# AI4REALNET/network-distributed-q-learning

Hardware: AMD Instinct MI355X
Metric: agent-env-steps/sec (whole node), 64-switch map, 1/2/4/8 MI355X vs CPU (higher is better)
Workload: dtype f64

## Files before the change

### network-distributed-q-learning_amd/csrc/sfl_core.h

```cpp
#pragma once
#include <stdint.h>
#include "sfl_rng.h"

#if !defined(__HIPCC__)
#include <math.h>
#endif

namespace sfl {

enum : uint32_t { A_NOTHING = 0, A_LEFT = 1, A_FWD = 2, A_RIGHT = 3, A_STOP = 4, A_NONE = 15 };
enum : uint32_t { S_WAITING = 0, S_READY = 1, S_MF_OFF = 2, S_MOVING = 3, S_STOPPED = 4, S_MALF = 5, S_DONE = 6 };
enum : int32_t { PH_RESET = 0, PH_TICK = 1, PH_DECIDE = 2, PH_POST = 3, PH_END = 4 };
enum : uint32_t { F_TERM = 1, F_TRUNC = 2, F_GREEDY = 4, F_EXPLOIT_DONE = 8, F_OWN_SCAN = 16, F_INFLIGHT = 32 };
enum : uint32_t { F_EXT_OBS = 128 };
enum : uint32_t {
  E_INF_DIST = 1,
  E_PLAN_OVF = 2,
  E_PORT = 4,
  E_BAD_ACTION = 8,
  E_LR_TABLE = 32,
};

constexpr int32_t DIST_INF = 0x3FFFFFFF;
constexpr int OWN_MAX = 16;
constexpr int MAXW = 4;
constexpr uint32_t PEND_NONE = 0xFFFFFFFFu;
constexpr uint16_t PORT_NONE = 0xFFFFu;

struct SflMap {
  int32_t H, W, S, T, K, NP, HW, cell_bits;
  int32_t max_episode_steps, mf_min, mf_max, ntab;
  int32_t delay_thr;
  double mf_rate, gamma, eps0, eps_decay, lr0, lr_decay, default_q;
  uint64_t mf_thresh, mf_magic;
  uint32_t mf_n;
  int64_t max_steps;
  uint64_t q_per_env;
  uint32_t rows_per_env, touched_words;
  const uint16_t* grid;
  const int16_t* cell_sw;
  const uint8_t* sw_np;
  const uint8_t* sw_na;
  const uint8_t* act_src;
  const uint8_t* act_dst;
  const uint8_t* act_turn;
  const uint8_t* act_j;
  const uint8_t* first_other;
  const uint8_t* port_side;
  const uint8_t* slot_nroutes;
  const uint8_t* slot_route_act;
  const uint8_t* q_w;
  const int16_t* port_nb;
  const int16_t* port_len;
  const int16_t* port_unique;
  const uint64_t* q_off;
  const uint32_t* row_base;
  const int32_t* dist;
  const int32_t* tr_ed;
  const int32_t* tr_la;
  const int32_t* tr_k;
  const int32_t* tr_target;
  const int32_t* tr_init_cell;
  const int32_t* tr_init_dist;
  const int32_t* tr_init_delay;
  const uint8_t* tr_init_dir;
  const int16_t* tr_init_port;
  const double* eps_tab;
  const double* lr_tab;
  const uint32_t* sw_pack;
  const uint32_t* port_pack;
  const uint32_t* move_tab;
  const uint32_t* move2c_tab;
  const int32_t* tr_pack;
  const uint32_t* seedseq32;
  const uint32_t* port_tr;
  const uint8_t* mf_tab;
  int32_t mf_steps;
  int32_t n_groups;
  const uint16_t* env_group;
  const double* hpg_eps_tab;
  const double* hpg_lr_tab;
  const double* hpg_sc;
};
enum : int { HPG_EPS0 = 0, HPG_EPS_DECAY = 1, HPG_LR0 = 2, HPG_LR_DECAY = 3 };

SFL_FN uint32_t mod_small(uint64_t x, uint32_t n, uint64_t M) {
#if defined(__HIP_DEVICE_COMPILE__)
  const uint64_t q = __umul64hi(x, M);
#else
  const uint64_t q = (uint64_t)(((unsigned __int128)x * M) >> 64);
#endif
  uint64_t r = x - q * (uint64_t)n;
  if (r >= n) r -= n;
  return (uint32_t)r;
}

inline void mf_prepare(SflMap& m) {
  const double R = ldexp(m.mf_rate, 53);
  m.mf_thresh = !(m.mf_rate > 0.0) ? 0ull : (R >= 9007199254740992.0 ? (1ull << 53) : (uint64_t)ceil(R));
  const int64_t n = (int64_t)m.mf_max - (int64_t)m.mf_min + 1;
  m.mf_n = (n >= 1 && n < (1ll << 32)) ? (uint32_t)n : 0u;
  m.mf_magic = m.mf_n ? ~0ull / m.mf_n : 0ull;
}

SFL_FN uint32_t mf_propose(const SflMap& m, uint64_t seed, uint32_t e, int32_t t, int h) {
  if (m.mf_steps > 0) {
    if (t < 1 || t > m.mf_steps) return 0u;
    return m.mf_tab[((size_t)e * (uint32_t)m.mf_steps + (uint32_t)(t - 1)) * (uint32_t)m.T + (uint32_t)h];
  }
  if (!(m.mf_rate > 0.0)) return 0u;
  const uint64_t z = mf_draw(seed, (uint64_t)t, (uint64_t)h);
  if ((z >> 11) >= m.mf_thresh) return 0u;
  const uint64_t x = mix64(z ^ 0xA0761D6478BD642Full);
  const uint32_t r = m.mf_n ? mod_small(x, m.mf_n, m.mf_magic)
                            : (uint32_t)(x % (uint64_t)(m.mf_max - m.mf_min + 1));
  return (uint32_t)(m.mf_min + (int32_t)r) + 1u;
}

struct SflState {
  uint32_t E;
  int32_t* phase;
  int32_t* elapsed;
  uint32_t* eflags;
  int32_t* ep_t;
  int32_t* n_test;
  uint32_t* epoch;
  uint64_t* rng;
  uint64_t* seed;
  double* cum_reward;
  int32_t* n_mf;
  int32_t* ep_dec;
  int32_t* ep_ticks;
  int64_t* step_ctr;
  int64_t* dec_total;
  uint32_t* masks;
  uint32_t* err;
  int32_t* tr_pos;
  uint32_t* tr_bits;
  uint32_t* tr_plan;
  uint16_t* tr_next;
  uint16_t* tr_prev;
  uint16_t* tr_src;
  uint16_t* tr_dec;
  int32_t* tr_delay;
  uint16_t* own;
  uint8_t* own_n;
  int32_t* sc_desired;
  int32_t* sc_pred;
  uint32_t* sc_aux;
  uint8_t* occ;
  uint8_t* claim;
  uint64_t* sem;
  uint64_t* slot;
  uint32_t* counts;
  double* q;
  uint32_t* touched;
};

struct SflCtl {
  int32_t mode;
  int32_t exploit_freq;
  int32_t ep_target;
  int32_t stats_cap;
  int32_t stats_base;
  int64_t dec_budget;
  double* st_cum;
  int32_t* st_arrived;
  int32_t* st_mf;
  int32_t* st_dec;
  int32_t* st_ticks;
  int32_t* st_delays;
  double* sx_cum;
  int32_t* sx_arrived;
  uint64_t* launch_dec;
  uint64_t* launch_ticks;
  uint64_t* launch_bytes;
  uint64_t* trace;
  uint64_t* trace_n;
  int32_t trace_env;
  int32_t trace_cap;
  const struct SflExt* ext;
  uint64_t* phase_cyc;
};

struct SflExt {
  const int32_t* actions;
  int32_t* agent;
  int32_t* train;
  int32_t* slot;
  uint32_t* state;
  uint32_t* mask;
  int32_t* reward;
  int32_t* now;
  int32_t* next_sw;
  int32_t* step_now;
  uint32_t* arrived;
  int32_t* n_mf;
  int32_t* delays;
  int32_t* truncated;
// ... 1248 lines not shown
```

### network-distributed-q-learning_amd/csrc/sfl_engine.h

```cpp
#pragma once
#include <stdint.h>
#include <stdio.h>
#include <stdlib.h>
#include <string.h>

#include <algorithm>
#include <string>
#include <vector>

#include "../../include/sfl.h"
#include "sfl_consensus.h"
#include "sfl_core.h"
#include "sfl_curve.h"
#include "sfl_mfgen.h"
#include "sfl_part.h"

namespace sfl {

static thread_local std::string g_last_error;

inline int fail(const std::string& msg) {
  g_last_error = msg;
  return -1;
}
// ... 626 lines not shown
  if (write) h->eblk_state = 0;
  return 0;
}

template <class B>
int scan_errors(Handle<B>* h) {
  if (!h->last_err) return 0;
  if (int rc = part_host_access(h, false)) return rc;
  std::vector<uint32_t> err(h->E);
  h->be.d2h(err.data(), h->st.err, h->E * 4);
  if (h->be.sync()) return fail(h->be.error());
  for (uint32_t e = 0; e < h->E; ++e)
    if (err[e]) {
      char buf[256];
      snprintf(buf, sizeof buf, "env %u: error flags 0x%x (1=inf distance, 2=plan overflow, 4=port mismatch, 8=bad action, "
               "16=message segment overflow, 32=decayed lr beyond the ntab table: raise ntab)",
               e, err[e]);
      return fail(buf);
    }
  return 0;
}

template <class B>
int check_errors(Handle<B>* h) {
  if (int rc = reduce_launch(h)) return rc;
  return scan_errors(h);
}

template <class B>
int run(Handle<B>* h, const SflCtl& c_in, sfl_run_args* args) {
  if (h->part.world) return fail("sfl_run: the handle is graph-partitioned; drive it with sfl_part_*");
  if (h->env_mode) return fail("sfl_run: the handle is in external-action mode (sfl_env_begin); drive it with sfl_env_step");
  const bool grouped = h->map.env_group != nullptr;
  if (grouped && args && args->trace && args->trace_cap > 0)
    return fail("sfl_run: a per-decision trace is not available on a handle with hyperparameter groups");
  SflCtl c = c_in;
  const size_t E = h->E, T = h->map.T;
  const int32_t cap = args ? args->stats_cap : 0;
  std::vector<void*> scratch;
  auto scr = [&](size_t bytes) -> void* {
    void* p = h->be.alloc(bytes ? bytes : 1);
    scratch.push_back(p);
    return p;
  };
  c.stats_cap = cap;
  c.stats_base = c_in.stats_base;
  if (args && cap > 0) {
    c.st_cum = (double*)scr((size_t)cap * E * 8);
    c.st_arrived = (int32_t*)scr((size_t)cap * E * 4);
    c.st_mf = (int32_t*)scr((size_t)cap * E * 4);
    c.st_dec = (int32_t*)scr((size_t)cap * E * 4);
    c.st_ticks = (int32_t*)scr((size_t)cap * E * 4);
    c.st_delays = (int32_t*)scr((size_t)cap * T * E * 4);
    c.sx_cum = (double*)scr((size_t)cap * E * 8);
    c.sx_arrived = (int32_t*)scr((size_t)cap * E * 4);
    for (void* p : scratch)
      if (!p) {
        for (void* q : scratch) h->be.free(q);
        return fail("sfl_run: stats allocation failed");
      }
    h->be.memset(c.sx_cum, 0, (size_t)cap * E * 8);
    h->be.memset(c.sx_arrived, 0, (size_t)cap * E * 4);
  }
  const bool curve = !args && h->cv.on;
  if (curve) {
    const CurveArgs& a = h->cv.a;
    c.stats_cap = a.ring_cap;
    c.stats_base = 0;
    c.st_cum = const_cast<double*>(a.st_cum);
    c.st_arrived = const_cast<int32_t*>(a.st_arrived);
    c.st_mf = const_cast<int32_t*>(a.st_mf);
    c.st_dec = const_cast<int32_t*>(a.st_dec);
    c.st_ticks = const_cast<int32_t*>(a.st_ticks);
    c.st_delays = const_cast<int32_t*>(a.st_delays);
  }
  const bool xfold = curve && h->cv.x_on;
  if (xfold) {
    c.sx_cum = const_cast<double*>(h->cv.xa.sx_cum);
    c.sx_arrived = const_cast<int32_t*>(h->cv.xa.sx_arrived);
  }
  c.launch_dec = h->d_launch_dec;
  c.launch_ticks = h->d_launch_ticks;
  c.launch_bytes = h->d_launch_bytes;
  c.phase_cyc = args && !grouped ? h->d_phase : nullptr;
  uint64_t* d_trace = nullptr;
  uint64_t* d_trace_n = nullptr;
  if (args && args->trace && args->trace_cap > 0) {
    d_trace = (uint64_t*)scr((size_t)args->trace_cap * 32);
    d_trace_n = (uint64_t*)scr(8);
    if (!d_trace || !d_trace_n) {
      for (void* q : scratch) h->be.free(q);
      return fail("sfl_run: trace allocation failed");
    }
    h->be.memset(d_trace_n, 0, 8);
    c.trace = d_trace;
    c.trace_n = d_trace_n;
    c.trace_env = args->trace_env;
    c.trace_cap = args->trace_cap;
  }
  float ms = 0.f;
  int rc = h->be.run(h->map, h->st, c, h->variant, &ms);
  h->last_kernel_ms = ms;
  if (!rc && curve) rc = h->be.curve(h->cv.a, false);
  if (!rc && xfold) rc = h->be.curve_exploit(h->cv.xa, false);
  if (!rc && args && cap > 0) {
    if (args->cum_reward) h->be.d2h(args->cum_reward, c.st_cum, (size_t)cap * E * 8);
    if (args->arrived) h->be.d2h(args->arrived, c.st_arrived, (size_t)cap * E * 4);
    if (args->malfunctions) h->be.d2h(args->malfunctions, c.st_mf, (size_t)cap * E * 4);
    if (args->decisions) h->be.d2h(args->decisions, c.st_dec, (size_t)cap * E * 4);
    if (args->ticks) h->be.d2h(args->ticks, c.st_ticks, (size_t)cap * E * 4);
    if (args->delays) h->be.d2h(args->delays, c.st_delays, (size_t)cap * T * E * 4);
    if (args->exploit_cum) h->be.d2h(args->exploit_cum, c.sx_cum, (size_t)cap * E * 8);
    if (args->exploit_arrived) h->be.d2h(args->exploit_arrived, c.sx_arrived, (size_t)cap * E * 4);
  }
  if (!rc && d_trace) {
    h->be.d2h(args->trace_n, d_trace_n, 8);
    h->be.d2h(args->trace, d_trace, (size_t)args->trace_cap * 32);
  }
  if (!rc) rc = h->be.sync();
  for (void* p : scratch) h->be.free(p);
  if (rc) return fail(std::string("sfl_run: ") + h->be.error());
  if (curve) {
    h->cv.last_ms = h->be.elapsed_ms();
    h->cv.x_last_ms = xfold ? h->be.elapsed_exploit_ms() : 0.f;
    h->cv.last_ms += h->cv.x_last_ms;
    h->cv.total_ms += h->cv.last_ms;
    h->cv.x_total_ms += h->cv.x_last_ms;
  }
  return check_errors(h);
}

inline int ext_variant(int v) {
  if (v <= 0 || !kVariants[v].LM) return v;
  for (int u = 1; u < kNumVariants; ++u) {
    const WaveShape &a = kVariants[u], &b = kVariants[v];
    if (!a.LM && a.PPL == b.PPL && a.SPL == b.SPL && a.TW == b.TW && a.G == b.G) return u;
  }
  return 0;
}

template <class B>
int env_begin(Handle<B>* h, bool wave = false) {
  const std::string fn = wave ? "sfl_env_begin_wave" : "sfl_env_begin";
  if (h->part.world) return fail(fn + ": the handle is graph-partitioned");
  if (h->map.env_group) return fail(fn + ": the handle has hyperparameter groups (sfl_set_hparam_groups)");
  int variant = 0;
  if (wave) {
    if (!B::kHasWave)
      return fail(fn + ": this build has no wave kernels (the host build runs the lane-per-env body only)");
    variant = ext_variant(h->created_variant);
    if (variant <= 0)
      return fail(fn + ": the handle has no wave shape (" +
                  (h->variant_note.empty() ? std::string("SFL_KERNEL=scalar") : h->variant_note) + ")");
  }
  const size_t E = h->E, T = h->map.T, S = h->map.S, NP = h->map.NP;
  if (!h->d_ext) {
    SflExt& x = h->ext;
    x.actions = h->template dalloc<int32_t>(E);
    x.agent = h->template dalloc<int32_t>(E);
    x.train = h->template dalloc<int32_t>(E);
    x.slot = h->template dalloc<int32_t>(E);
    x.state = h->template dalloc<uint32_t>(E);
    x.mask = h->template dalloc<uint32_t>(E);
    x.reward = h->template dalloc<int32_t>(E);
    x.now = h->template dalloc<int32_t>(E);
    x.next_sw = h->template dalloc<int32_t>(E);
    x.step_now = h->template dalloc<int32_t>(E);
// ... 792 lines not shown
```

### network-distributed-q-learning_amd/csrc/sfl_rng.h

```cpp
#pragma once
#include <stdint.h>

#ifndef SFL_FN
#if defined(__HIPCC__)
#define SFL_FN __host__ __device__ inline __attribute__((always_inline))
#else
#define SFL_FN inline
#endif
#endif

namespace sfl {

struct Pcg64 {
  uint64_t shi, slo;
  uint64_t ihi, ilo;
  uint32_t has;
  uint32_t buf;
};

SFL_FN uint64_t mulhi64(uint64_t a, uint64_t b) {
#if defined(__HIP_DEVICE_COMPILE__)
  return __umul64hi(a, b);
#else
  return (uint64_t)(((unsigned __int128)a * b) >> 64);
// ... 23 lines not shown
    return g.buf;
  }
  uint64_t v = pcg_next64(g);
  g.has = 1;
  g.buf = (uint32_t)(v >> 32);
  return (uint32_t)v;
}

SFL_FN double pcg_double(Pcg64& g) { return (double)(pcg_next64(g) >> 11) * (1.0 / 9007199254740992.0); }

SFL_FN uint32_t pcg_bounded(Pcg64& g, uint32_t rng) {
  if (rng == 0) return 0;
  if (rng == 0xFFFFFFFFu) return pcg_next32(g);
  const uint32_t excl = rng + 1u;
  uint64_t m = (uint64_t)pcg_next32(g) * excl;
  uint32_t left = (uint32_t)m;
  if (left < excl) {
    const uint32_t thr = (0xFFFFFFFFu - rng) % excl;
    while (left < thr) {
      m = (uint64_t)pcg_next32(g) * excl;
      left = (uint32_t)m;
    }
  }
  return (uint32_t)(m >> 32);
}

SFL_FN void pcg_from_seedseq(uint32_t value, Pcg64& g) {
  uint32_t hc = 0x43b0d7e5u;
  uint32_t pool[4];
  for (int i = 0; i < 4; ++i) {
    uint32_t v = (i == 0) ? value : 0u;
    v ^= hc;
    hc *= 0x931e8875u;
    v *= hc;
    v ^= v >> 16;
    pool[i] = v;
  }
  for (int src = 0; src < 4; ++src) {
    for (int dst = 0; dst < 4; ++dst) {
      if (src == dst) continue;
      uint32_t v = pool[src];
      v ^= hc;
      hc *= 0x931e8875u;
      v *= hc;
      v ^= v >> 16;
      uint32_t r = 0xca01f9ddu * pool[dst] - 0x4973f715u * v;
      r ^= r >> 16;
      pool[dst] = r;
    }
  }
  uint32_t w[8];
  uint32_t hb = 0x8b51f9ddu;
  for (int i = 0; i < 8; ++i) {
    uint32_t d = pool[i & 3];
    d ^= hb;
    hb *= 0x58f38dedu;
    d *= hb;
    d ^= d >> 16;
    w[i] = d;
  }
  const uint64_t s_hi = (uint64_t)w[0] | ((uint64_t)w[1] << 32);
  const uint64_t s_lo = (uint64_t)w[2] | ((uint64_t)w[3] << 32);
  const uint64_t q_hi = (uint64_t)w[4] | ((uint64_t)w[5] << 32);
  const uint64_t q_lo = (uint64_t)w[6] | ((uint64_t)w[7] << 32);
  g.ihi = (q_hi << 1) | (q_lo >> 63);
  g.ilo = (q_lo << 1) | 1ull;
  g.shi = 0;
  g.slo = 0;
  pcg_step(g);
  uint64_t lo = g.slo + s_lo;
  g.shi = g.shi + s_hi + (lo < g.slo ? 1ull : 0ull);
  g.slo = lo;
  pcg_step(g);
  g.has = 0;
  g.buf = 0;
}

SFL_FN uint64_t mix64(uint64_t z) {
  z = (z ^ (z >> 30)) * 0xBF58476D1CE4E5B9ull;
  z = (z ^ (z >> 27)) * 0x94D049BB133111EBull;
  return z ^ (z >> 31);
}

SFL_FN uint64_t mf_draw(uint64_t seed, uint64_t tick, uint64_t handle) {
  return mix64(seed * 0x9E3779B97F4A7C15ull + tick * 0xD1B54A32D192ED03ull + handle * 0x8CB92BA72F3D8DD7ull +
               0x632BE59BD9B4E019ull);
}

}
```

### network-distributed-q-learning_amd/csrc/sfl_wave.h

```cpp
#pragma once
#include <hip/hip_runtime.h>

#include <type_traits>

#include "sfl_core.h"
#include "sfl_part.h"
#include "sfl_experiment.h"

namespace sfl {
namespace wave {

#ifndef SFL_PF_RING
#define SFL_PF_RING 12
#endif
#ifndef SFL_PF_RING64
#define SFL_PF_RING64 16
#endif
#ifndef SFL_TICK_HOLD
#define SFL_TICK_HOLD 2
#endif
#ifndef SFL_TICK_REMMIN
#define SFL_TICK_REMMIN 5
#endif

// ... 854 lines not shown
          w[0] = mk;
          w[1] = 0ull;
        } else {
          w[0] = mk.w[0];
          w[1] = mk.w[1];
        }
#pragma unroll
        for (int j = 0; j < 2 * NWD; ++j) st(s.masks, (size_t)(k * MAXW + j) * E + e, (uint32_t)(w[j >> 1] >> (32 * (j & 1))));
      };
      put(0, q_mask);
      put(1, arr_mask);
      put(2, fl_mask);
      put(3, mf_mask);
      if constexpr (!EXT) {
        st(s.rng, ix(0), lrng[0]);
        st(s.rng, ix(1), lrng[1]);
        st(s.rng, ix(4), lrng[4]);
      }
      st(s.cum_reward, e, (double)cum);
      st(s.n_mf, e, n_mf);
      st(s.ep_dec, e, ep_dec);
      st(s.ep_ticks, e, ep_ticks);
      st(s.step_ctr, e, (int64_t)step_ctr);
      st(s.dec_total, e, ld(s.dec_total, e) + (int64_t)n_dec);
    }
    return err;
  }
  __device__ __forceinline__ void store_eblk(int32_t phase, uint32_t err, int32_t ep_t, int32_t n_test, int64_t dec_done,
                                             int32_t req_dst, uint32_t upd_n, uint64_t l_dec, uint64_t l_ticks,
                                             uint64_t l_bytes) {
    if constexpr (PART) {
      uint32_t* sg = lsem0;
      auto put4 = [&](int i, uint32_t a, uint32_t b, uint32_t c, uint32_t d) {
        u4 v;
        v[0] = a;
        v[1] = b;
        v[2] = c;
        v[3] = d;
        *(u4*)(sg + i) = v;
      };
      auto lo = [](uint64_t x) { return (uint32_t)x; };
      auto hi = [](uint64_t x) { return (uint32_t)(x >> 32); };
      const uint64_t dtot = ebw64(EB_DEC_TOTAL) + (uint64_t)n_dec;
      const uint64_t cumd = (uint64_t)__double_as_longlong((double)cum);
      const uint64_t r0 = lrng[0], r1 = lrng[1], r2 = lrng[2], r3 = lrng[3], r4 = lrng[4];
      uint64_t mw[4][2];
      auto mwords = [&](int k, const Mask& mk) {
        if constexpr (TPL * G <= 64 || TWc <= 32) {
          mw[k][0] = (uint64_t)mk;
          mw[k][1] = 0ull;
        } else {
          mw[k][0] = mk.w[0];
          mw[k][1] = mk.w[1];
        }
      };
      mwords(0, q_mask);
      mwords(1, arr_mask);
      mwords(2, fl_mask);
      mwords(3, mf_mask);
      static_assert(EB_PHASE == 0 && EB_EP_DEC == 8 && EB_STEP_CTR == 10 && EB_RNG == 16 && EB_MASKS == 26 &&
                        EB_DEC_DONE == 42 && EB_USED == 52 && MAXW == 4,
                    "block layout");
      put4(0, (uint32_t)phase, (uint32_t)now, flags, epoch);
      put4(4, err, (uint32_t)ep_t, (uint32_t)n_test, (uint32_t)n_mf);
      put4(8, (uint32_t)ep_dec, (uint32_t)ep_ticks, (uint32_t)step_ctr, 0u);
      put4(12, lo(dtot), hi(dtot), lo(cumd), hi(cumd));
      put4(16, lo(r0), hi(r0), lo(r1), hi(r1));
      put4(20, lo(r2), hi(r2), lo(r3), hi(r3));
      put4(24, lo(r4), hi(r4), lo(mw[0][0]), hi(mw[0][0]));
      put4(28, lo(mw[0][1]), hi(mw[0][1]), lo(mw[1][0]), hi(mw[1][0]));
      put4(32, lo(mw[1][1]), hi(mw[1][1]), lo(mw[2][0]), hi(mw[2][0]));
      put4(36, lo(mw[2][1]), hi(mw[2][1]), lo(mw[3][0]), hi(mw[3][0]));
      put4(40, lo(mw[3][1]), hi(mw[3][1]), lo((uint64_t)dec_done), hi((uint64_t)dec_done));
      put4(44, (uint32_t)req_dst, upd_n, lo(l_dec), hi(l_dec));
      put4(48, lo(l_ticks), hi(l_ticks), lo(l_bytes), hi(l_bytes));
      const uint32_t v = sg[lane < EB_USED ? lane : 0];
      if (lane < EB_USED) st(P->eblk, (size_t)e * PART_EB + (uint32_t)lane, v);
    }
  }

  __device__ __forceinline__ void reset() {
    now = 0;
#pragma unroll
    for (int k = 0; k < TPL; ++k) {
      if (mine[k]) {
        const int hk = lane + G * k;
        const uint32_t t_init = (uint32_t)ltt[8 * hk + 7];
        pos[k] = -1;
        bits[k] = tb_make(t_init & 0xFFu, S_WAITING, A_NONE, 0, 0, 0);
        plan[k] = 0;
        nprv[k] = (nprv[k] & 0xFFFF0000u) | (t_init >> 16);
        delay[k] = ltt[8 * hk + 6];
      }
    }
#pragma unroll
    for (int k = 0; k < PPL; ++k) sem(k) = 0u;
    for (int h = 0; h < m.T; ++h) {
      const vec_t<int32_t, 8> tr = LDCV<vec_t<int32_t, 8>>(m.tr_pack, (size_t)h);
      sset((int)((uint32_t)tr[7] >> 16), r_pack(h, 1, tr[0] - 2, tr[0] + tr[5]));
    }
    flags &= ~(F_TERM | F_TRUNC | F_OWN_SCAN | F_INFLIGHT);
    q_mask = arr_mask = fl_mask = mf_mask = Mask{};
    malf_keep(Mask{});
    epoch = (epoch + 1u) & 0xFFu;
    if (epoch == 0) {
      for (int i = lane; i < m.S * m.T; i += G) st(sbase(), (size_t)i, slot_make(PEND_NONE, 0, 0));
      epoch = 1;
    }
    cum = 0;
    n_mf = 0;
    ep_dec = 0;
    ep_ticks = 0;
    step_ctr = 0;
  }

  __device__ __forceinline__ void tick() {
    PrioGuard<PART ? 0 : SFL_SETPRIO_TICK> prio;
    if constexpr (xp::kNoTick) {
      ++now;
      return;
    }
    pf_ok = false;
    const int32_t t = ++now;
    const uint64_t seed = s.seed[e];
    vec_t<int32_t, 4> tt0[TPL], tt1[TPL];
#pragma unroll
    for (int k = 0; k < TPL; ++k) {
      tt0[k] = *(const vec_t<int32_t, 4>*)(ltt + 8 * (mine_(k) ? lid() + G * k : 0));
      tt1[k] = *(const vec_t<int32_t, 4>*)(ltt + 8 * (mine_(k) ? lid() + G * k : 0) + 4);
    }
    u4 mrows[TPL];
#pragma unroll
    for (int k = 0; k < TPL; ++k) {
      const bool ok = mine_(k);
      const int pc = pos[k] >= 0 ? pos[k] : tt1[k][0];
      const int pd = pos[k] >= 0 ? (int)tb_dir(bits[k]) : (int)((uint32_t)tt1[k][3] & 0xFFu);
      mrows[k] = move_row((uint32_t)(ok ? pc : 0) * 4u + (uint32_t)(ok ? pd : 0));
    }
    bool mover[TPL];
    int32_t desired[TPL], pred[TPL];
    uint32_t aux[TPL];
#pragma unroll
    for (int k = 0; k < TPL; ++k) {
      const int h = lid() + G * k;
      const int32_t t_init_cell = tt1[k][0];
      const uint32_t t_init_dir = (uint32_t)tt1[k][3] & 0xFFu;
      mover[k] = false;
      desired[k] = -1;
      pred[k] = -1;
      aux[k] = 0;
      if (mine_(k)) {
        const uint32_t b = bits[k];
        const int32_t p0 = pos[k];
        uint32_t st_ = tb_state(b), dir = tb_dir(b), prev = tb_prev(b), saved = tb_saved(b), mf = tb_mf(b);
        uint32_t given = A_NOTHING;
        pred[k] = p0;
        const int pc = p0 >= 0 ? p0 : t_init_cell;
        const int pd = p0 >= 0 ? (int)dir : (int)t_init_dir;
        const u4 mrow = mrows[k];
        auto mv_of = [&](uint32_t a) -> Move {
          const uint32_t q = a & 3u;
          return unpack_move(q == 0 ? mrow[0] : q == 1 ? mrow[1] : q == 2 ? mrow[2] : mrow[3]);
        };
        if (!tb_done(b)) {
          const uint32_t pl = plan[k];
          if (pl_len(pl) == 0) {
            given = A_FWD;
          } else {
            given = pl_front(pl);
            prev = given;
            plan[k] = pl_pop(pl);
          }
          if (p0 >= 0) {
            const Move mv = mv_of(given);
            aux[k] |= 1u << 12;
            if (mv.valid) {
              aux[k] |= 1u << 13;
              pred[k] = mv.cell;
              if (dest_sw(mv) >= 0) aux[k] |= 1u << 14;
            }
          }
        }
        if (st_ != S_DONE && mf == 0) mf = mf_propose(m, seed, e, t, h);
        uint32_t pa = given;
        if (pa == A_NOTHING && st_ == S_MOVING) pa = A_FWD;
        if (st_ == S_WAITING) pa = A_NOTHING;
        if (pa == A_LEFT || pa == A_RIGHT) {
          const Move mv = mv_of(pa);
          if (!(mv.cell_ok && mv.valid)) pa = A_FWD;
        }
        if (is_moving_action(pa)) {
          const Move mv = mv_of(pa);
          if (!(mv.cell_ok && mv.valid)) pa = A_STOP;
        }
        if (is_moving_action(pa) && saved == 0 && st_ != S_DONE) saved = pa;
        const bool update_allowed = (mf == 0) && pa != A_STOP;
        desired[k] = p0;
        uint32_t ddir = dir;
        if (st_ == S_DONE) {
        } else if (p0 < 0 && saved != 0) {
          desired[k] = t_init_cell;
          ddir = t_init_dir;
          mover[k] = true;
        } else if (saved != 0 && update_allowed) {
          const Move mv = mv_of(saved);
          desired[k] = mv.cell;
          ddir = (uint32_t)mv.dir;
          pa = saved;
          mover[k] = desired[k] != p0;
        }
        aux[k] |= pa | (ddir << 4) | (given << 8);
        bits[k] = tb_make(dir, st_, prev, saved, mf, tb_done(b));
      }
    }
    const Mask M = mbal(mover);
    Mask A{};
    if (many(M)) {
      bool onmap[TPL];
#pragma unroll
      for (int k = 0; k < TPL; ++k) onmap[k] = mine_(k) && pos[k] >= 0;
      Mask same[TPL], occs[TPL];
      const Mask occ0 = mbal(onmap);
#pragma unroll
      for (int k = 0; k < TPL; ++k) {
        same[k] = M;
        occs[k] = occ0;
      }
      for (int bi = 0; bi < m.cell_bits; ++bi) {
        bool pd_[TPL], pp_[TPL];
#pragma unroll
        for (int k = 0; k < TPL; ++k) {
          pd_[k] = mover[k] && (((uint32_t)desired[k] >> bi) & 1u);
          pp_[k] = onmap[k] && (((uint32_t)pos[k] >> bi) & 1u);
        }
        const Mask bd = mbal(pd_), bp = mbal(pp_);
#pragma unroll
        for (int k = 0; k < TPL; ++k) {
          const bool one = ((uint32_t)desired[k] >> bi) & 1u;
          same[k] &= one ? bd : ~bd;
          occs[k] &= one ? bp : ~bp;
        }
      }
      if (m.cell_bits < 32) {
        bool pn[TPL];
#pragma unroll
        for (int k = 0; k < TPL; ++k) pn[k] = mover[k] && desired[k] < 0;
        const Mask bd = mbal(pn);
#pragma unroll
        for (int k = 0; k < TPL; ++k) {
          same[k] &= desired[k] < 0 ? bd : ~bd;
          if (desired[k] < 0) occs[k] = Mask{};
        }
      }
      bool win[TPL];
      int occ[TPL];
#pragma unroll
      for (int k = 0; k < TPL; ++k) {
        const int h = lid() + G * k;
        win[k] = mover[k] && !many(same[k] & mbelow(Mask{}, h));
        const Mask occset = occs[k] & ~mone(Mask{}, h);
        occ[k] = (mover[k] && many(occset)) ? mhighest(occset) : -1;
      }
      while (true) {
        bool cand[TPL];
#pragma unroll
        for (int k = 0; k < TPL; ++k) {
          const int h = lid() + G * k;
          cand[k] = mover[k] && win[k] && !mbit(A, h) && (occ[k] < 0 || (mbit(M, occ[k]) && mbit(A, occ[k])));
        }
        const Mask nb = mbal(cand);
        if (!many(nb)) break;
        A |= nb;
      }
    }
    const bool over = t >= m.max_episode_steps;
    bool done[TPL], newdone[TPL], isdone[TPL], newly[TPL], dep[TPL];
#pragma unroll
    for (int k = 0; k < TPL; ++k) {
      const int h = lid() + G * k;
      const int32_t t_ed = tt0[k][0], t_target = tt0[k][3], t_init_cell = tt1[k][0];
      const uint32_t t_init_dir = (uint32_t)tt1[k][3] & 0xFFu;
      done[k] = false;
      isdone[k] = !mine_(k);
      newly[k] = false;
      newdone[k] = false;
      dep[k] = false;
      if (mine_(k)) {
        const uint32_t b = bits[k];
        const int32_t p0 = pos[k];
        uint32_t st_ = tb_state(b), dir = tb_dir(b), saved = tb_saved(b), mf = tb_mf(b);
        const uint32_t pa = aux[k] & 15u;
        const bool in_mf = mf > 0;
        bool ma = in_mf ? false : (mover[k] && mbit(A, h));
        const bool valid_move = is_moving_action(pa) && ma;
        const bool ed_reached = t >= t_ed;
        const uint32_t prev_st = st_;
// ... 945 lines not shown
        w[1] = arr_mask.w[1];
      }
#pragma unroll
      for (int j = 0; j < MAXW; ++j) st(x.arrived, (size_t)j * E + e, (uint32_t)(w[j >> 1] >> (32 * (j & 1))));
      if (c.launch_dec) st(c.launch_dec, e, (uint64_t)(applied ? 1u : 0u));
      if (c.launch_ticks) st(c.launch_ticks, e, (uint64_t)ticks);
      if (c.launch_bytes) st(c.launch_bytes, e, (uint64_t)0);
    }
    return phase;
  }
};

enum { TM_TICK = 0, TM_OBS = 1, TM_EG = 2, TM_APPLY = 3, TM_POST = 4, TM_RESET = 5, TM_OTHER = 6, TM_TOTAL = 7 };
constexpr uint32_t TM_SAMPLE = 8;
struct PhaseTimer {
  bool on;
  uint64_t t, acc[8];
  __device__ __forceinline__ void start(bool on_) {
    on = on_;
    t = on ? (uint64_t)__builtin_amdgcn_s_memtime() : 0ull;
#pragma unroll
    for (int k = 0; k < 8; ++k) acc[k] = 0ull;
    acc[TM_TOTAL] = t;
  }
  __device__ __forceinline__ void lap(int k) {
    if (on) {
      const uint64_t n = (uint64_t)__builtin_amdgcn_s_memtime();
      acc[k] += n - t;
      t = n;
    }
  }
  template <class V>
  __device__ __forceinline__ void decide_done(const V& v, int lane) {
    if (on) {
      const uint64_t n = (uint64_t)__builtin_amdgcn_s_memtime();
      if (lane >= 0) {
        const uint64_t o = ((uint64_t)(uint32_t)__builtin_amdgcn_readlane((int)(v.tm_obs_t >> 32), lane) << 32) |
                           (uint32_t)__builtin_amdgcn_readlane((int)(uint32_t)v.tm_obs_t, lane);
        const uint64_t g = ((uint64_t)(uint32_t)__builtin_amdgcn_readlane((int)(v.tm_eg_t >> 32), lane) << 32) |
                           (uint32_t)__builtin_amdgcn_readlane((int)(uint32_t)v.tm_eg_t, lane);
        acc[TM_OBS] += o - t;
        acc[TM_EG] += g - o;
        acc[TM_APPLY] += n - g;
      } else {
        acc[TM_OTHER] += n - t;
      }
      t = n;
    }
  }
  __device__ __forceinline__ void flush(const SflCtl& c) {
    if (!on) return;
    const uint64_t end = (uint64_t)__builtin_amdgcn_s_memtime();
    acc[TM_TOTAL] = end - acc[TM_TOTAL];
    uint64_t known = 0;
#pragma unroll
    for (int k = 0; k < 6; ++k) known += acc[k];
    acc[TM_OTHER] = acc[TM_TOTAL] > known ? acc[TM_TOTAL] - known : 0ull;
    if (__lane_id() == 0)
#pragma unroll
      for (int k = 0; k < 8; ++k) atomicAdd((unsigned long long*)&c.phase_cyc[k], (unsigned long long)acc[k]);
  }
};

template <int PPL, int SPL, int TW, bool TRACE, bool PART = false, bool TIMED = false, bool HPG = false, bool EXT = false>
__device__ void run(const SflMap& m, const SflState& s, const SflCtl& c, const SflPart* P = nullptr) {
  static_assert(!(EXT && (TRACE || TIMED)), "external-action mode: no trace, no phase timers");
  using V = WEnv<PPL, SPL, TW, PART, 64, false, HPG, EXT>;
  constexpr int LDS_WORDS =
      64 * (PPL + SPL) + V::PF_SLOTS * PF_WORDS + 12 + (PART ? 64 * PPL + 2 * SPL + 6 * 64 * V::TPL : TW * 8);
  const int lane = (int)__lane_id();
  const uint32_t e = uni((uint32_t)((blockIdx.x * blockDim.x + threadIdx.x) >> 6));
  if (e >= s.E) return;
  constexpr int WPB = TW > 64 ? 1 : SFL_WAVE_BLOCK / 64;
  __shared__ uint32_t lds[WPB * LDS_WORDS];
  V v(m, s, e, lane, lds + (threadIdx.x >> 6) * LDS_WORDS, P);
  if constexpr (PART) {
    v.lsem0 = lds + (threadIdx.x >> 6) * LDS_WORDS + 64 * (PPL + SPL) + V::PF_SLOTS * PF_WORDS + 12;
    v.ldirty = v.lsem0 + 64 * PPL;
    v.ltr0 = v.ldirty + 2 * SPL;
  }
  PhaseTimer tm;
  if constexpr (TIMED) tm.start(c.phase_cyc != nullptr && blockIdx.x % TM_SAMPLE == 0u);
  v.load();
  if constexpr (EXT) {
    v.store(v.ext_run(c, uni(ld(s.phase, e))));
    return;
  }
  if constexpr (PART)
    if (v.flags & F_DEFER) return;
  if constexpr (xp::kLoadTwice) v.load();
  const int64_t dec_base = PART ? (int64_t)v.ebw64(EB_DEC_DONE) : 0;
  int32_t phase = PART ? (int32_t)v.ebw(EB_PHASE) : uni(ld(s.phase, e));
  int32_t ep_t = PART ? (int32_t)v.ebw(EB_EP_T) : uni(ld(s.ep_t, e));
  int32_t n_test = PART ? (int32_t)v.ebw(EB_N_TEST) : uni(ld(s.n_test, e));
  uint32_t ticks = 0, abytes = 0;
  typename V::Dec d;
  const bool test_mode = c.mode == 1;
  const int64_t max_steps = m.max_steps, dec_budget = c.dec_budget;
  while (true) {
    if (phase == PH_RESET) {
      if (test_mode) {
        if (c.ep_target >= 0 && n_test >= c.ep_target) break;
        v.flags |= F_GREEDY;
      } else {
        if (c.ep_target >= 0 && ep_t >= c.ep_target) break;
        if (c.exploit_freq > 0 && (ep_t + 1) % c.exploit_freq == 0 && !(v.flags & F_EXPLOIT_DONE)) v.flags |= F_GREEDY;
        else v.flags &= ~F_GREEDY;
      }
      if constexpr (TIMED) tm.lap(TM_OTHER);
      v.reset();
      if constexpr (TIMED) tm.lap(TM_RESET);
      phase = PH_TICK;
    } else if (phase == PH_TICK) {
      abytes += 36u * (uint32_t)(m.T - mpopc(v.arr_mask));
      if constexpr (TIMED) tm.lap(TM_OTHER);
      v.tick();
      if constexpr (TIMED) tm.lap(TM_TICK);
      ticks++;
      phase = v.after_tick();
    } else if (phase == PH_DECIDE || phase == PH_POST) {
      const bool greedy = (v.flags & F_GREEDY) != 0;
      auto finish = [&]() -> bool {
        if constexpr (TIMED) tm.lap(TM_OTHER);
        v.post(d, greedy);
        if constexpr (TIMED) tm.lap(TM_POST);
        if (TRACE && c.trace && (int32_t)e == c.trace_env) v.trace_decision(c, d, lane);
        v.count_decision(d, max_steps);
        phase = v.after_post();
        return dec_budget > 0 && dec_base + (int64_t)v.n_dec >= dec_budget;
      };
      bool stop = false, do_decide = phase == PH_DECIDE;
      while (true) {
        if (do_decide) {
          if (PART && !(v.flags & F_REQ) && dec_budget > 0 && dec_base + (int64_t)v.n_dec >= dec_budget) {
            stop = true;
            break;
          }
          if constexpr (TIMED) {
            tm.lap(TM_OTHER);
            v.tm_on = tm.on;
          }
          const bool requested = v.template decide<TIMED>(d, greedy);
          if constexpr (TIMED) tm.decide_done(v, 0);
          if (PART && requested) {
            stop = true;
            break;
          }
          abytes += d.abytes;
          v.flags |= F_INFLIGHT;
          if (!many(v.q_mask)) {
            phase = PH_TICK;
            break;
          }
        }
        do_decide = true;
        stop = finish();
        if (stop || phase != PH_DECIDE) break;
      }
      if (stop) break;
    } else {
      const int arrived = mpopc(v.arr_mask);
      const size_t cap = (size_t)(c.stats_cap > 0 ? c.stats_cap : 1);
      const bool greedy = (v.flags & F_GREEDY) != 0;
      if (c.st_cum && c.stats_cap > 0 && (!greedy || test_mode)) {
        const int32_t idx = (greedy && test_mode) ? n_test : ep_t;
        const size_t row = (size_t)(idx - c.stats_base) % cap;
        if (lane == 0) {
          st(c.st_cum, row * s.E + e, (double)v.cum);
          st(c.st_arrived, row * s.E + e, (int32_t)arrived);
          st(c.st_mf, row * s.E + e, v.n_mf);
          st(c.st_dec, row * s.E + e, v.ep_dec);
          st(c.st_ticks, row * s.E + e, v.ep_ticks);
        }
#pragma unroll
        for (int k = 0; k < V::TPL; ++k)
          if (v.mine[k]) st(c.st_delays, (row * m.T + lane + V::kG * k) * s.E + e, v.delay[k]);
      }
      if (greedy && !test_mode && c.sx_cum && c.stats_cap > 0 && lane == 0) {
        const size_t row = (size_t)(ep_t - c.stats_base) % cap;
        st(c.sx_cum, row * s.E + e, (double)v.cum);
        st(c.sx_arrived, row * s.E + e, (int32_t)arrived);
      }
      if (greedy) {
        if (test_mode) n_test += 1;
        else v.flags |= F_EXPLOIT_DONE;
      } else {
        ep_t += 1;
        v.flags &= ~F_EXPLOIT_DONE;
      }
      phase = PH_RESET;
    }
  }
  const uint32_t err_out = v.store(phase);
  if constexpr (xp::kStoreTwice) v.store(phase);
  if constexpr (PART)
    v.store_eblk(phase, err_out, ep_t, n_test, dec_base + (int64_t)v.n_dec, v.req_dst_v,
                 v.n_upd < P->upd_env ? v.n_upd : P->upd_env, (uint64_t)v.n_dec, (uint64_t)ticks, (uint64_t)abytes);
  if constexpr (TIMED) tm.flush(c);
  if constexpr (!PART) v.store_launch(c, ep_t, n_test, ticks, abytes, lane);
}

template <int PPL, int SPL, int TW, bool TRACE, int G, bool TIMED = false, bool LM = false, bool HPG = false, bool EXT = false>
__device__ void run_groups(const SflMap& m, const SflState& s, const SflCtl& c) {
  static_assert(!(EXT && (TRACE || TIMED)), "external-action mode: no trace, no phase timers");
  using V = WEnv<PPL, SPL, TW, false, G, LM, HPG, EXT>;
  constexpr int LDS_WORDS = (G * (PPL + SPL) + V::PF_SLOTS * PF_WORDS + 12 + 3) / 4 * 4;
  constexpr int EPB = SFL_GROUP_BLOCK / G;
  constexpr int SWX = G * SPL, NPX = G * PPL;
  constexpr int O_TT = EPB * LDS_WORDS, O_SW = O_TT + TW * 8, O_PP = O_SW + SWX * V::SW_LDS, O_PT = O_PP + NPX * 4;
  constexpr int O_LM = O_PT + NPX * 4, LM_WORDS = LM ? 16128 : 0;
  static_assert(!LM || 2 * (O_LM + LM_WORDS) * 4 <= 163840, "LM: two blocks' LDS exceed a CU's 160 KB");
  __shared__ __attribute__((aligned(16))) uint32_t lds[O_LM + LM_WORDS];
  for (int i = (int)threadIdx.x; i < m.S * V::SW_LDS; i += (int)blockDim.x)
    lds[O_SW + i] = m.sw_pack[(i / V::SW_LDS) * 16 + i % V::SW_LDS];
  for (int i = (int)threadIdx.x; i < m.NP * 4; i += (int)blockDim.x) {
    lds[O_PP + i] = m.port_pack[i];
    lds[O_PT + i] = m.port_tr[i];
  }
  const int lm_mv = LM ? m.HW * 16 : 0;
  if constexpr (LM) {
    const int nd = m.K * m.HW * 4;
    for (int i = (int)threadIdx.x; i < lm_mv; i += (int)blockDim.x) lds[O_LM + i] = m.move_tab[i];
    for (int j = (int)threadIdx.x; 2 * j < nd; j += (int)blockDim.x) {
      const uint32_t lo = d16(m.dist[2 * j]), hi = 2 * j + 1 < nd ? d16(m.dist[2 * j + 1]) : 0u;
      lds[O_LM + lm_mv + j] = lo | (hi << 16);
    }
  }
  __syncthreads();
  const uint32_t e = (uint32_t)((blockIdx.x * blockDim.x + threadIdx.x) / G);
  if (e >= s.E) return;
  V v(m, s, e, (int)__lane_id(), lds + (threadIdx.x / G) * LDS_WORDS, nullptr, (int32_t*)(lds + O_TT));
  v.tsw = lds + O_SW;
  v.tpp = lds + O_PP;
  v.tpt = lds + O_PT;
  if constexpr (LM) {
    v.lmv = lds + O_LM;
    v.ldist = lds + O_LM + lm_mv;
  }
  PhaseTimer tm;
  if constexpr (TIMED) tm.start(c.phase_cyc != nullptr && blockIdx.x % TM_SAMPLE == 0u && threadIdx.x < 64u);
  v.load();
  if constexpr (EXT) {
    v.store(v.ext_run(c, ld(s.phase, e)));
    return;
  }
  int32_t phase = ld(s.phase, e);
  int32_t ep_t = ld(s.ep_t, e), n_test = ld(s.n_test, e);
  uint32_t ticks = 0, abytes = 0;
  typename V::Dec d;
  const bool test_mode = c.mode == 1;
  const int32_t max_steps = m.max_steps < 0x7FFFFFFF ? (int32_t)m.max_steps : 0x7FFFFFFF;
  const uint32_t dec_budget = c.dec_budget > 0 ? (c.dec_budget < 0xFFFFFFFFll ? (uint32_t)c.dec_budget : 0xFFFFFFFFu) : 0xFFFFFFFFu;
  while (true) {
    if (phase == PH_RESET) {
      bool target = false;
      if (test_mode) {
        target = c.ep_target >= 0 && n_test >= c.ep_target;
        v.flags |= F_GREEDY;
      } else {
        target = c.ep_target >= 0 && ep_t >= c.ep_target;
        if (c.exploit_freq > 0 && (ep_t + 1) % c.exploit_freq == 0 && !(v.flags & F_EXPLOIT_DONE)) v.flags |= F_GREEDY;
        else v.flags &= ~F_GREEDY;
      }
      if (target) break;
      v.reset();
      phase = PH_TICK;
    }
    if constexpr (TIMED) tm.lap(TM_RESET);
    const bool dec_ph = phase == PH_POST || phase == PH_DECIDE;
    const bool wave_decides = (int)__builtin_popcountll(__ballot(dec_ph)) >= SFL_TICK_HOLD * G &&
                              (SFL_TICK_REMMIN <= 0 || __ballot(dec_ph && mpopc(v.q_mask) < SFL_TICK_REMMIN) != 0ull);
    if constexpr (TIMED) tm.lap(TM_OTHER);
    if (phase == PH_TICK && !wave_decides) {
      abytes += 36u * (uint32_t)(m.T - mpopc(v.arr_mask));
      v.tick();
      ticks++;
      phase = v.after_tick();
    }
    if constexpr (TIMED) tm.lap(TM_TICK);
    if (phase == PH_POST) {
      const bool greedy = (v.flags & F_GREEDY) != 0;
      v.post(d, greedy);
      if (TRACE && c.trace && (int32_t)e == c.trace_env) v.trace_decision(c, d, v.lane);
      v.count_decision(d, max_steps);
      phase = v.after_post();
      if (v.n_dec >= dec_budget) break;
    }
    if constexpr (TIMED) {
      tm.lap(TM_POST);
      v.tm_on = tm.on;
    }
    const uint64_t dec_lanes = TIMED ? (uint64_t)__ballot(phase == PH_DECIDE) : 0ull;
    if (phase == PH_DECIDE) {
      const bool greedy = (v.flags & F_GREEDY) != 0;
      v.template decide<TIMED>(d, greedy);
      abytes += d.abytes;
      v.flags |= F_INFLIGHT;
      phase = many(v.q_mask) ? PH_POST : PH_TICK;
    }
    if constexpr (TIMED) tm.decide_done(v, dec_lanes ? __builtin_ctzll(dec_lanes) : -1);
    if (phase == PH_END) {
      const int arrived = mpopc(v.arr_mask);
      const size_t cap = (size_t)(c.stats_cap > 0 ? c.stats_cap : 1);
      const bool greedy = (v.flags & F_GREEDY) != 0;
      if (c.st_cum && c.stats_cap > 0 && (!greedy || test_mode)) {
        const int32_t idx = (greedy && test_mode) ? n_test : ep_t;
        const size_t row = (size_t)(idx - c.stats_base) % cap;
        if (v.lane == 0) {
          st(c.st_cum, row * s.E + e, (double)v.cum);
          st(c.st_arrived, row * s.E + e, (int32_t)arrived);
          st(c.st_mf, row * s.E + e, v.n_mf);
          st(c.st_dec, row * s.E + e, v.ep_dec);
          st(c.st_ticks, row * s.E + e, v.ep_ticks);
        }
#pragma unroll
        for (int k = 0; k < V::TPL; ++k)
          if (v.mine[k]) st(c.st_delays, (row * m.T + v.lane + G * k) * s.E + e, v.delay[k]);
      }
      if (greedy && !test_mode && c.sx_cum && c.stats_cap > 0 && v.lane == 0) {
        const size_t row = (size_t)(ep_t - c.stats_base) % cap;
        st(c.sx_cum, row * s.E + e, (double)v.cum);
        st(c.sx_arrived, row * s.E + e, (int32_t)arrived);
      }
      if (greedy) {
        if (test_mode) n_test += 1;
        else v.flags |= F_EXPLOIT_DONE;
      } else {
        ep_t += 1;
        v.flags &= ~F_EXPLOIT_DONE;
      }
      phase = PH_RESET;
    }
  }
  v.store(phase);
  if constexpr (TIMED) tm.flush(c);
  v.store_launch(c, ep_t, n_test, ticks, abytes, v.lane);
// ... 5 lines not shown
```

Baseline: 1.709 billion.

## Branch-free tick step, hoisted malfunction hash base, and parallel reset seeding

The per-train tick logic becomes a branch-free select chain, which cuts divergence across the wavefront. The malfunction random draw now hoists the seed/tick hash base out of the per-train loop and only computes durations for the rare hits, one at a time under a wave ballot. Reset moves the semaphore seeding into each lane's owned trains using LDS atomic max when G<64, replacing the serial loop over all trains. It also adds timer laps and a compile flag for phase timing, and the parallel reset relies on atomic-max ordering matching the old sequential writes.

```diff
diff --git a/network-distributed-q-learning_amd/csrc/sfl_core.h b/network-distributed-q-learning_amd/csrc/sfl_core.h
--- a/network-distributed-q-learning_amd/csrc/sfl_core.h
+++ b/network-distributed-q-learning_amd/csrc/sfl_core.h
@@ -103,6 +103,14 @@
   m.mf_magic = m.mf_n ? ~0ull / m.mf_n : 0ull;
 }
 
+SFL_FN bool mf_hit(const SflMap& m, uint64_t z) { return (z >> 11) < m.mf_thresh; }
+SFL_FN uint32_t mf_duration(const SflMap& m, uint64_t z) {
+  const uint64_t x = mix64(z ^ 0xA0761D6478BD642Full);
+  const uint32_t r = m.mf_n ? mod_small(x, m.mf_n, m.mf_magic)
+                            : (uint32_t)(x % (uint64_t)(m.mf_max - m.mf_min + 1));
+  return (uint32_t)(m.mf_min + (int32_t)r) + 1u;
+}
+
 SFL_FN uint32_t mf_propose(const SflMap& m, uint64_t seed, uint32_t e, int32_t t, int h) {
   if (m.mf_steps > 0) {
     if (t < 1 || t > m.mf_steps) return 0u;
@@ -110,11 +118,7 @@
   }
   if (!(m.mf_rate > 0.0)) return 0u;
   const uint64_t z = mf_draw(seed, (uint64_t)t, (uint64_t)h);
-  if ((z >> 11) >= m.mf_thresh) return 0u;
-  const uint64_t x = mix64(z ^ 0xA0761D6478BD642Full);
-  const uint32_t r = m.mf_n ? mod_small(x, m.mf_n, m.mf_magic)
-                            : (uint32_t)(x % (uint64_t)(m.mf_max - m.mf_min + 1));
-  return (uint32_t)(m.mf_min + (int32_t)r) + 1u;
+  return mf_hit(m, z) ? mf_duration(m, z) : 0u;
 }
 
 struct SflState {
diff --git a/network-distributed-q-learning_amd/csrc/sfl_engine.h b/network-distributed-q-learning_amd/csrc/sfl_engine.h
--- a/network-distributed-q-learning_amd/csrc/sfl_engine.h
+++ b/network-distributed-q-learning_amd/csrc/sfl_engine.h
@@ -732,7 +732,11 @@
   c.launch_dec = h->d_launch_dec;
   c.launch_ticks = h->d_launch_ticks;
   c.launch_bytes = h->d_launch_bytes;
+#ifdef SFL_STEP_TIMED
+  c.phase_cyc = !grouped ? h->d_phase : nullptr;
+#else
   c.phase_cyc = args && !grouped ? h->d_phase : nullptr;
+#endif
   uint64_t* d_trace = nullptr;
   uint64_t* d_trace_n = nullptr;
   if (args && args->trace && args->trace_cap > 0) {
diff --git a/network-distributed-q-learning_amd/csrc/sfl_rng.h b/network-distributed-q-learning_amd/csrc/sfl_rng.h
--- a/network-distributed-q-learning_amd/csrc/sfl_rng.h
+++ b/network-distributed-q-learning_amd/csrc/sfl_rng.h
@@ -129,9 +129,12 @@
   return z ^ (z >> 31);
 }
 
+SFL_FN uint64_t mf_draw_base(uint64_t seed, uint64_t tick) {
+  return seed * 0x9E3779B97F4A7C15ull + tick * 0xD1B54A32D192ED03ull + 0x632BE59BD9B4E019ull;
+}
+SFL_FN uint64_t mf_draw_at(uint64_t base, uint64_t handle) { return mix64(base + handle * 0x8CB92BA72F3D8DD7ull); }
 SFL_FN uint64_t mf_draw(uint64_t seed, uint64_t tick, uint64_t handle) {
-  return mix64(seed * 0x9E3779B97F4A7C15ull + tick * 0xD1B54A32D192ED03ull + handle * 0x8CB92BA72F3D8DD7ull +
-               0x632BE59BD9B4E019ull);
+  return mf_draw_at(mf_draw_base(seed, tick), handle);
 }
 
 }
diff --git a/network-distributed-q-learning_amd/csrc/sfl_wave.h b/network-distributed-q-learning_amd/csrc/sfl_wave.h
--- a/network-distributed-q-learning_amd/csrc/sfl_wave.h
+++ b/network-distributed-q-learning_amd/csrc/sfl_wave.h
@@ -960,22 +960,31 @@
   __device__ __forceinline__ void reset() {
     now = 0;
 #pragma unroll
+    for (int k = 0; k < PPL; ++k) sem(k) = 0u;
+    static_assert(R_OWNER_SHIFT + 7 == 30, "the owner is the record's highest field below `in`");
+#pragma unroll
     for (int k = 0; k < TPL; ++k) {
-      if (mine[k]) {
-        const int hk = lane + G * k;
-        const uint32_t t_init = (uint32_t)ltt[8 * hk + 7];
+      if (mine_(k)) {
+        const int hk = lid() + G * k;
+        const vec_t<int32_t, 4> row = *(const vec_t<int32_t, 4>*)(ltt + 8 * hk + 4);
+        const uint32_t t_init = (uint32_t)row[3];
         pos[k] = -1;
         bits[k] = tb_make(t_init & 0xFFu, S_WAITING, A_NONE, 0, 0, 0);
         plan[k] = 0;
         nprv[k] = (nprv[k] & 0xFFFF0000u) | (t_init >> 16);
-        delay[k] = ltt[8 * hk + 6];
-      }
-    }
-#pragma unroll
-    for (int k = 0; k < PPL; ++k) sem(k) = 0u;
-    for (int h = 0; h < m.T; ++h) {
-      const vec_t<int32_t, 8> tr = LDCV<vec_t<int32_t, 8>>(m.tr_pack, (size_t)h);
-      sset((int)((uint32_t)tr[7] >> 16), r_pack(h, 1, tr[0] - 2, tr[0] + tr[5]));
+        delay[k] = row[2];
+        if constexpr (G < 64) {
+          const int32_t ed = ltt[8 * hk];
+          __hip_atomic_fetch_max(lsem + (t_init >> 16), r_pack((uint32_t)hk, 1, ed - 2, ed + row[1]), __ATOMIC_RELAXED,
+                                 __HIP_MEMORY_SCOPE_WORKGROUP);
+        }
+      }
+    }
+    if constexpr (G == 64) {
+      for (int h = 0; h < m.T; ++h) {
+        const vec_t<int32_t, 8> tr = LDCV<vec_t<int32_t, 8>>(m.tr_pack, (size_t)h);
+        sset((int)((uint32_t)tr[7] >> 16), r_pack(h, 1, tr[0] - 2, tr[0] + tr[5]));
+      }
     }
     flags &= ~(F_TERM | F_TRUNC | F_OWN_SCAN | F_INFLIGHT);
     q_mask = arr_mask = fl_mask = mf_mask = Mask{};
@@ -1015,81 +1024,94 @@
       const int pd = pos[k] >= 0 ? (int)tb_dir(bits[k]) : (int)((uint32_t)tt1[k][3] & 0xFFu);
       mrows[k] = move_row((uint32_t)(ok ? pc : 0) * 4u + (uint32_t)(ok ? pd : 0));
     }
+    uint32_t mfn[TPL];
+#pragma unroll
+    for (int k = 0; k < TPL; ++k) mfn[k] = 0u;
+    if (m.mf_steps > 0) {
+#pragma unroll
+      for (int k = 0; k < TPL; ++k)
+        if (mine_(k) && tb_state(bits[k]) != S_DONE && tb_mf(bits[k]) == 0) mfn[k] = mf_propose(m, seed, e, t, lid() + G * k);
+    } else if (m.mf_rate > 0.0) {
+      const uint64_t zb = mf_draw_base(seed, (uint64_t)t);
+      uint64_t z[TPL];
+      bool hit[TPL], todo = false;
+#pragma unroll
+      for (int k = 0; k < TPL; ++k) {
+        z[k] = mf_draw_at(zb, (uint64_t)(lid() + G * k));
+        hit[k] = mine_(k) && tb_state(bits[k]) != S_DONE && tb_mf(bits[k]) == 0 && mf_hit(m, z[k]);
+        todo |= hit[k];
+      }
+      while (__ballot(todo) != 0ull) {
+        bool first[TPL], seen = false;
+        uint64_t zz = z[0];
+#pragma unroll
+        for (int k = 0; k < TPL; ++k) {
+          first[k] = hit[k] && !seen;
+          seen |= hit[k];
+          zz = first[k] ? z[k] : zz;
+        }
+        const uint32_t dur = mf_duration(m, zz);
+        todo = false;
+#pragma unroll
+        for (int k = 0; k < TPL; ++k) {
+          mfn[k] = first[k] ? dur : mfn[k];
+          hit[k] = hit[k] && !first[k];
+          todo |= hit[k];
+        }
+      }
+    }
     bool mover[TPL];
     int32_t desired[TPL], pred[TPL];
     uint32_t aux[TPL];
 #pragma unroll
     for (int k = 0; k < TPL; ++k) {
-      const int h = lid() + G * k;
       const int32_t t_init_cell = tt1[k][0];
       const uint32_t t_init_dir = (uint32_t)tt1[k][3] & 0xFFu;
-      mover[k] = false;
-      desired[k] = -1;
-      pred[k] = -1;
-      aux[k] = 0;
-      if (mine_(k)) {
-        const uint32_t b = bits[k];
-        const int32_t p0 = pos[k];
-        uint32_t st_ = tb_state(b), dir = tb_dir(b), prev = tb_prev(b), saved = tb_saved(b), mf = tb_mf(b);
-        uint32_t given = A_NOTHING;
-        pred[k] = p0;
-        const int pc = p0 >= 0 ? p0 : t_init_cell;
-        const int pd = p0 >= 0 ? (int)dir : (int)t_init_dir;
-        const u4 mrow = mrows[k];
-        auto mv_of = [&](uint32_t a) -> Move {
-          const uint32_t q = a & 3u;
-          return unpack_move(q == 0 ? mrow[0] : q == 1 ? mrow[1] : q == 2 ? mrow[2] : mrow[3]);
-        };
-        if (!tb_done(b)) {
-          const uint32_t pl = plan[k];
-          if (pl_len(pl) == 0) {
-            given = A_FWD;
-          } else {
-            given = pl_front(pl);
-            prev = given;
-            plan[k] = pl_pop(pl);
-          }
-          if (p0 >= 0) {
-            const Move mv = mv_of(given);
-            aux[k] |= 1u << 12;
-            if (mv.valid) {
-              aux[k] |= 1u << 13;
-              pred[k] = mv.cell;
-              if (dest_sw(mv) >= 0) aux[k] |= 1u << 14;
-            }
-          }
-        }
-        if (st_ != S_DONE && mf == 0) mf = mf_propose(m, seed, e, t, h);
-        uint32_t pa = given;
-        if (pa == A_NOTHING && st_ == S_MOVING) pa = A_FWD;
-        if (st_ == S_WAITING) pa = A_NOTHING;
-        if (pa == A_LEFT || pa == A_RIGHT) {
-          const Move mv = mv_of(pa);
-          if (!(mv.cell_ok && mv.valid)) pa = A_FWD;
-        }
-        if (is_moving_action(pa)) {
-          const Move mv = mv_of(pa);
-          if (!(mv.cell_ok && mv.valid)) pa = A_STOP;
-        }
-        if (is_moving_action(pa) && saved == 0 && st_ != S_DONE) saved = pa;
-        const bool update_allowed = (mf == 0) && pa != A_STOP;
-        desired[k] = p0;
-        uint32_t ddir = dir;
-        if (st_ == S_DONE) {
-        } else if (p0 < 0 && saved != 0) {
-          desired[k] = t_init_cell;
-          ddir = t_init_dir;
-          mover[k] = true;
-        } else if (saved != 0 && update_allowed) {
-          const Move mv = mv_of(saved);
-          desired[k] = mv.cell;
-          ddir = (uint32_t)mv.dir;
-          pa = saved;
-          mover[k] = desired[k] != p0;
-        }
-        aux[k] |= pa | (ddir << 4) | (given << 8);
-        bits[k] = tb_make(dir, st_, prev, saved, mf, tb_done(b));
-      }
+      const bool ok = mine_(k);
+      const uint32_t b = bits[k];
+      const int32_t p0 = pos[k];
+      const uint32_t st_ = tb_state(b), dir = tb_dir(b), saved0 = tb_saved(b), mf0 = tb_mf(b);
+      const bool live = !tb_done(b);
+      const u4 mrow = mrows[k];
+      auto word_of = [&](uint32_t a) -> uint32_t {
+        const uint32_t q = a & 3u;
+        return q == 0 ? mrow[0] : q == 1 ? mrow[1] : q == 2 ? mrow[2] : mrow[3];
+      };
+      auto usable = [](uint32_t w) { return ((w >> 22) & 3u) == 3u; };
+      const uint32_t w_fwd = mrow[A_FWD & 3u];
+      const uint32_t pl = plan[k];
+      const bool has = live && pl_len(pl) != 0;
+      const uint32_t given = live ? (has ? pl_front(pl) : (uint32_t)A_FWD) : (uint32_t)A_NOTHING;
+      const uint32_t prev = has ? given : tb_prev(b);
+      plan[k] = (ok && has) ? pl_pop(pl) : pl;
+      const uint32_t wg = word_of(given);
+      const Move mg = unpack_move(wg);
+      const bool onm = live && p0 >= 0;
+      const bool pv = onm && mg.valid;
+      const bool psw = pv && dest_sw(mg) >= 0;
+      pred[k] = ok ? (pv ? mg.cell : p0) : -1;
+      const uint32_t mf = (st_ != S_DONE && mf0 == 0) ? mfn[k] : mf0;
+      const bool to_fwd = given == A_NOTHING && st_ == S_MOVING;
+      uint32_t pa = to_fwd ? (uint32_t)A_FWD : given;
+      uint32_t wp = to_fwd ? w_fwd : wg;
+      pa = st_ == S_WAITING ? (uint32_t)A_NOTHING : pa;
+      const bool lr_off = (pa == A_LEFT || pa == A_RIGHT) && !usable(wp);
+      pa = lr_off ? (uint32_t)A_FWD : pa;
+      wp = lr_off ? w_fwd : wp;
+      pa = (is_moving_action(pa) && !usable(wp)) ? (uint32_t)A_STOP : pa;
+      const bool save = is_moving_action(pa) && saved0 == 0 && st_ != S_DONE;
+      const uint32_t saved = save ? pa : saved0;
+      const Move ms = unpack_move(save ? wp : word_of(saved0));
+      const bool act = st_ != S_DONE && saved != 0;
+      const bool dep = act && p0 < 0;
+      const bool go = act && p0 >= 0 && mf == 0 && pa != A_STOP;
+      const int32_t des = dep ? t_init_cell : go ? ms.cell : p0;
+      const uint32_t ddir = dep ? t_init_dir : go ? (uint32_t)ms.dir : dir;
+      pa = go ? saved : pa;
+      mover[k] = ok && (dep || (go && des != p0));
+      desired[k] = ok ? des : -1;
+      aux[k] = ok ? (pa | (ddir << 4) | (given << 8) | ((uint32_t)onm << 12) | ((uint32_t)pv << 13) | ((uint32_t)psw << 14)) : 0u;
+      bits[k] = ok ? tb_make(dir, st_, prev, saved, mf, tb_done(b)) : b;
     }
     const Mask M = mbal(mover);
     Mask A{};
@@ -2201,6 +2223,7 @@
   PhaseTimer tm;
   if constexpr (TIMED) tm.start(c.phase_cyc != nullptr && blockIdx.x % TM_SAMPLE == 0u);
   v.load();
+  if constexpr (TIMED) tm.lap(TM_OTHER);
   if constexpr (EXT) {
     v.store(v.ext_run(c, uni(ld(s.phase, e))));
     return;
@@ -2359,6 +2382,7 @@
   PhaseTimer tm;
   if constexpr (TIMED) tm.start(c.phase_cyc != nullptr && blockIdx.x % TM_SAMPLE == 0u && threadIdx.x < 64u);
   v.load();
+  if constexpr (TIMED) tm.lap(TM_OTHER);
   if constexpr (EXT) {
     v.store(v.ext_run(c, ld(s.phase, e)));
     return;
@@ -2371,6 +2395,7 @@
   const int32_t max_steps = m.max_steps < 0x7FFFFFFF ? (int32_t)m.max_steps : 0x7FFFFFFF;
   const uint32_t dec_budget = c.dec_budget > 0 ? (c.dec_budget < 0xFFFFFFFFll ? (uint32_t)c.dec_budget : 0xFFFFFFFFu) : 0xFFFFFFFFu;
   while (true) {
+    if constexpr (TIMED) tm.lap(TM_OTHER);
     if (phase == PH_RESET) {
       bool target = false;
       if (test_mode) {
```

After: 1.716 billion (median of 6 runs). About the same (+0.4%).
